# proroklab/magat_pathplanning

Measured on AMD Instinct MI355X. Metric: agent-steps/s (batched GAT forward), higher is better.
Workload: dtype f32 in/out, fp32-class arithmetic: convolutions + GAT maps as f16x3 split products on the 16-bit matrix cores with f32 accumulation (the encoder head too, on the layer3 kernel's pooled map; with GAT_MFMA the attention scores and the K-hop aggregation as well), MLPs on f32 MFMA

## Files before the change

### magat_pathplanning_amd/_native.py

```python
import ctypes
import os
import threading

PKG = os.path.dirname(os.path.abspath(__file__))
LIB_PATH = os.environ.get("MAGAT_LIB_PATH") or os.path.join(PKG, "lib", "libmagat_hip.so")

MODE_KEYQUERY = 0
MODE_GAT_MODIFIED = 1
MODE_GAT_ORIGIN = 2
MODE_GNN = 3
_MODE_IDS = {"KeyQuery": MODE_KEYQUERY, "GAT_modified": MODE_GAT_MODIFIED, "GAT_origin": MODE_GAT_ORIGIN}
TAGS = {0: "untagged", 1: "conv_first", 2: "layer1.conv1", 3: "layer1.conv2+ds", 4: "layer2.conv1",
        5: "layer2.conv2+ds", 6: "layer3.conv1", 7: "layer3.conv2+ds", 8: "head(avgpool+fc+linear)",
        9: "compressMLP", 10: "gat_maps_gemm", 11: "gat_graph", 12: "actionsMLP", 13: "head_mean",
        14: "gat_pack", 15: "gso_prepare", 16: "gat_prepare", 17: "range_guard", 18: "layer1.conv2+layer2 (fused)", 19: "gat_layer (one launch)", 20: "gso_to_csr", 21: "gat_cast", 22: "layer3 (fused, pooled)", 23: "layer1.conv2+layer2+layer3 (fused, pooled)", 24: "conv_wgrad", 25: "gnn_dense", 26: "sim_guided", 27: "sim_expert", 28: "sim_mapf", 29: "sim_mapf_lns", 30: "sim_mapf_audit", 31: "sim_mapf_cbs", 32: "sim_mapf_ecbs"}
TAG_ACTIONS = 12
FORMS = {"head_longk": 0, "head_splitk": 1, "gat_pack": 2, "gat_persist": 3, "gat_hsplit": 4, "chain_persist": 5,
         "head_compress": 6, "guard_one": 7, "csr_fused": 8, "gat_mid": 9, "chain_lat": 10, "head_lat": 11, "guard_lat": 12, "stem_lat": 13, "actions_tail": 14, "gnn_dense": 15, "sim_guided": 16, "sim_expert": 17, "sim_mapf": 18, "sim_mapf_lns": 19, "sim_mapf_audit": 20, "sim_mapf_cbs": 21, "sim_mapf_ecbs": 22}
TAG_GNN_DENSE = 25
TAG_SIM_GUIDED = 26
TAG_SIM_EXPERT = 27
TAG_SIM_MAPF = 28
TAG_SIM_MAPF_LNS = 29
TAG_SIM_MAPF_AUDIT = 30
TAG_SIM_MAPF_CBS = 31
TAG_SIM_MAPF_ECBS = 32
GUIDE_LOCAL, GUIDE_GLOBAL, GUIDE_SEMI = 1, 2, 3

_lock = threading.Lock()
_lib = None


class MagatNativeError(RuntimeError):
# ... 215 lines not shown
```

### magat_pathplanning_amd/csrc/block_fused.hip

```cpp
#include "magat_common.h"

namespace {
#ifndef MAGAT_CHAIN_NT
#define MAGAT_CHAIN_NT 3
#endif
#if MAGAT_CHAIN_NT & 1
#define MAGAT_CHAIN_NT_STR " nt"
#else
#define MAGAT_CHAIN_NT_STR ""
#endif
#if MAGAT_CHAIN_NT & 2
#define CHAIN_OUT_STORE(ptr, val) __builtin_nontemporal_store((val), reinterpret_cast<f32x4*>(ptr))
#else
#define CHAIN_OUT_STORE(ptr, val) (*reinterpret_cast<f32x4*>(ptr) = (val))
#endif
#include "block_walk.h"
struct ChainParams {
  const char* in1;
  const char* in2;
  char* out;
  int out_gl;
  long long out_pix_stride, out_tile;
  const char* wA; const char* wB; const char* wC;
  const float* bA; const float* bB; const float* bC;
// ... 349 lines not shown
    __syncthreads();
    CHAIN_STAMP(3);
    if (more) dma_map(p.in1, group + (int)gridDim.x, LDS_X1N);
    if (rg == 0) chain_stage4<W4A, 32, 0, 64, false>(p, lds, LDS_Y, 0, LDS_Z, p.wB, ct, p.bB, sB, group, clamped);
    else chain_stage4<W4B, 32, 0, 64, false>(p, lds, LDS_Y, 0, LDS_Z, p.wB, ct, p.bB, sB, group, clamped);
    CHAIN_STAMP(4);
    __syncthreads();
    CHAIN_STAMP(5);
    if (rg == 0) chain_stage4<W4A, 64, 32, 64, true>(p, lds, LDS_Z, LDS_Y, 0, p.wC, ct, p.bC, sC, group, clamped);
    else chain_stage4<W4B, 64, 32, 64, true>(p, lds, LDS_Z, LDS_Y, 0, p.wC, ct, p.bC, sC, group, clamped);
    CHAIN_STAMP(6);
  }
  if (clamped && p.range_flag) atomicOr(p.range_flag, 1);
}

struct FullParams { ChainParams c; L3Params l; };



__global__ __launch_bounds__(256, 1) void block_full_p_kernel(const FullParams q) {
  extern __shared__ __attribute__((aligned(1024))) char lds[];
  const ChainParams& p = q.c;
  const L3Params& l3 = q.l;
  const int t = threadIdx.x, lane = t & 63;
  const int wave = __builtin_amdgcn_readfirstlane(t >> 6);
  for (int i = t; i < 32 * (PIXB / 4); i += 256)
    *reinterpret_cast<unsigned*>(lds + (i / (PIXB / 4)) * BLK + ZPIX * PIXB + (i % (PIXB / 4)) * 4) = 0u;
  auto dma_map = [&](const char* base, int group, int lds_off, int first, int step, int last) {
    const int m0 = group * AG;
    const long long tile_b = (long long)(m0 >> 7) * NPIX * (128 * 32 * 4) + (m0 & 127) * 16;
    for (int item = first; item < last; item += step) {
      const int blk = item / 5, part = item % 5;
      const int pix = part * 8 + (lane >> 3);
      const char* src = base + tile_b + (long long)pix * (128 * 32 * 4) + (blk >> 2) * (256 * 32) + (blk & 3) * 2048 +
                        (lane & 7) * 16;
      const unsigned m0v = __builtin_amdgcn_readfirstlane((unsigned)(uintptr_t)lds + (unsigned)(lds_off + blk * BLK + part * 8 * PIXB));
      if (pix < NPIX) asm volatile("s_mov_b32 m0, %1\n\tglobal_load_lds_dwordx4 %0, off" MAGAT_CHAIN_NT_STR ::"v"(src), "s"(m0v) : "memory", "m0");
    }
  };
  const float sA = *p.sA, sB = *p.sB, sC = *p.sC, s1 = *l3.s1, s2 = *l3.s2;
  bool clamped = false;
  const int ct = wave & 1, rg = wave >> 1, ct2 = wave;
  constexpr int BPT1 = 9 * 4 * 2, BPT2A = 9 * 4 * 2, BPT2B = (9 * 4 + 4) * 2;
  f32x4 bq[4];
  {
    const int fh = lane >> 5;
#pragma unroll
    for (int qd = 0; qd < 4; ++qd) bq[qd] = *reinterpret_cast<const f32x4*>(l3.b2 + 32 * ct2 + 8 * qd + 4 * fh);
  }
  FULL_CLOCKS(0);
  const int gstride = (int)gridDim.x;
  constexpr int U0 = 0, U1 = MAP32, U2 = 2 * MAP32, U3 = 3 * MAP32;
  if ((int)blockIdx.x < p.groups) {
    dma_map(p.in1, blockIdx.x, U3, wave, 4, 40);
    dma_map(p.in2, blockIdx.x, U2, wave, 4, 40);
  }
#pragma unroll 1
  for (int group = blockIdx.x; group < p.groups; group += gstride) {
    const bool rows_ok = group * AG + ((lane & 31) & 7) < p.M;
    const bool more = group + gstride < p.groups;
// ... 7 lines not shown
      case 2: chain_stage4<W4P2, 32, 32, 32, false>(p, lds, U3, U2, U1, p.wA, 0, p.bA, sA, group, clamped); break;
      default: chain_stage4<W4P3, 32, 32, 32, false>(p, lds, U3, U2, U1, p.wA, 0, p.bA, sA, group, clamped); break;
    }
    __syncthreads();
    FULL_STAMP(2);
    if (rg == 0) chain_stage4<W4I, 32, 0, 64, false>(p, lds, U1, 0, U2, p.wB, ct, p.bB, sB, group, clamped);
    else chain_stage4<W4E, 32, 0, 64, false>(p, lds, U1, 0, U2, p.wB, ct, p.bB, sB, group, clamped);
    __syncthreads();
    FULL_STAMP(3);
    if (rg == 0) chain_stage4<W4I, 64, 32, 64, false, true>(p, lds, U2, U1, U0, p.wC, ct, p.bC, sC, group, clamped);
    else chain_stage4<W4E, 64, 32, 64, false, true>(p, lds, U2, U1, U0, p.wC, ct, p.bC, sC, group, clamped);
    __syncthreads();
    FULL_STAMP(4);
    constexpr int L_IN = U0, L_MID = U2;
    const int ct1 = ct, rg1 = rg;
    f32x16 acc[9];
#pragma unroll
    for (int s = 0; s < 9; ++s)
#pragma unroll
      for (int r = 0; r < 16; ++r) acc[s][r] = 0.f;
    auto l3_half = [&](const int h) __attribute__((always_inline)) {
      const char* w2 = h == 0 ? l3.w2a + (size_t)ct2 * BPT2A * 1024 : l3.w2b + (size_t)ct2 * BPT2B * 1024;
      const char* w1h = l3.w1 + (size_t)(2 * h) * BPT1 * 1024;
      if (rg1 == 0) {
        f32x16 a1[W4I::NT];
#pragma unroll
        for (int s = 0; s < W4I::NT; ++s)
#pragma unroll
          for (int r = 0; r < 16; ++r) a1[s][r] = 0.f;
        walk4<W4I, 4, 0, 8 * BLK, 8 * BLK, MAGAT_W4_D>(lds, L_IN, 0, w1h + (size_t)ct1 * BPT1 * 1024, a1, false);
        if (h == 0) FULL_STAMP(11); else FULL_STAMP(13);
        const int tl[W4I::NT] = {W4I::t[0], W4I::t[1], W4I::t[2], W4I::t[3]};
        epi_to_lds<64, W4I::NT>(lds, L_MID, tl, a1, ct1, l3.b1 + 64 * h, s1, rows_ok, clamped);
      } else {
        f32x16 a1[W4E::NT];
#pragma unroll
        for (int s = 0; s < W4E::NT; ++s)
#pragma unroll
          for (int r = 0; r < 16; ++r) a1[s][r] = 0.f;
        walk4<W4E, 4, 0, 8 * BLK, 8 * BLK, MAGAT_W4_D>(lds, L_IN, 0, w1h + (size_t)ct1 * BPT1 * 1024, a1, false);
        if (h == 0) FULL_STAMP(11); else FULL_STAMP(13);
        const int tl[W4E::NT] = {W4E::t[0], W4E::t[1], W4E::t[2], W4E::t[3], W4E::t[4]};
        epi_to_lds<64, W4E::NT>(lds, L_MID, tl, a1, ct1, l3.b1 + 64 * h, s1, rows_ok, clamped);
      }
      if (h == 0) FULL_STAMP(12); else FULL_STAMP(14);
      __syncthreads();
      FULL_STAMP(5 + 2 * h);
      walk4<W4All, 4, 4, 8 * BLK, 8 * BLK, MAGAT_W4_D>(lds, L_MID, L_IN, w2, acc, h == 1);
      L3_LDS_SYNC();
      FULL_STAMP(6 + 2 * h);
    };
#if defined(MAGAT_L3_UNROLL_H) && defined(MAGAT_DEBUG_HOOKS)
    l3_half(0);
    l3_half(1);
#else
#pragma unroll 1
    for (int h = 0; h < 2; ++h) l3_half(h);
#endif
    if (more) {
      dma_map(p.in1, group + gstride, U3, wave, 4, 40);
      dma_map(p.in2, group + gstride, U2, wave, 4, 40);
    }
    FULL_STAMP(9);
    {
      const int fr = lane & 31, fh = lane >> 5, agent = fr & 7;
      const bool lo = (lane >> 3) & 1, hi = (lane >> 4) & 1;
      const int m = group * AG + agent;
      const int cellF = 2 * (int)lo + 6 * (int)hi, cell0 = hi ? 1 : 7, cell1 = lo ? 3 : 5;
      float* ob = l3.out + (long long)(m >> 7) * 9 * (128 * 128) +
                  (l3.out_gl ? (8 * ct2 + fh) * 512 + (m & 127) * 4 : (m & 127) * 128 + 32 * ct2 + 4 * fh);
      const int qstep = l3.out_gl ? 1024 : 8;
      const bool mok = m < p.M;
#pragma unroll
      for (int qd = 0; qd < 4; ++qd) {
        f32x4 vF, v0, v1, v2;
#pragma unroll
        for (int c = 0; c < 4; ++c) {
          const int r = 4 * qd + c;
          float v[9];
// ... 99 lines not shown
  }
  const int grid = p.groups < cus ? p.groups : cus;
  hipLaunchKernelGGL(block3_w4_kernel, dim3((unsigned)grid), dim3(256), lds, st, p);
  magat_prof_end(pid, st);
  return magat_check_launch();
}

#ifdef MAGAT_DEBUG_HOOKS
extern "C" int magat_chain_set_debug_buffer(long long* dev_buf) { g_chain_dbg = dev_buf; return MAGAT_OK; }
extern "C" int magat_block3_set_debug_buffer(long long* dev_buf) { g_block3_dbg = dev_buf; return MAGAT_OK; }
#endif


int magat_block_full(const void* in1, const void* in2, const float* wchain, const float* bA, const float* bB, const float* bC,
                     float* out, const float* w3, const float* b1, const float* b2, int M, int* range_flag, hipStream_t st,
                     const float* scales, int out_gl) {
  if (!in1 || !in2 || !wchain || !bA || !bB || !bC || !out || !w3 || !b1 || !b2) return MAGAT_ERR_NULL;
  if (M <= 0) return MAGAT_ERR_BAD_SHAPE;
  FullParams q;
  ChainParams& p = q.c;
  p.in1 = static_cast<const char*>(in1); p.in2 = static_cast<const char*>(in2); p.out = nullptr;
  p.out_gl = 2; p.out_pix_stride = 0; p.out_tile = 0;
  const char* wb = reinterpret_cast<const char*>(wchain);
  const size_t nA = chain_block_bytes(32, 32, 32), nB = chain_block_bytes(32, 0, 64), nC = chain_block_bytes(64, 32, 64);
  p.wA = wb; p.wB = wb + nA + 16; p.wC = wb + nA + 16 + nB + 16;
  p.bA = bA; p.bB = bB; p.bC = bC;
  p.sA = reinterpret_cast<const float*>(p.wA + nA);
  p.sB = reinterpret_cast<const float*>(p.wB + nB);
  p.sC = reinterpret_cast<const float*>(p.wC + nC);
  p.M = M; p.groups = (M + AG - 1) / AG;
  p.range_flag = range_flag;
// ... 3 lines not shown
  const char* w3b = reinterpret_cast<const char*>(w3);
  const size_t n1 = (size_t)4 * 72 * 1024, n2a = (size_t)4 * 72 * 1024, n2b = (size_t)4 * 80 * 1024;
  l.w1 = w3b; l.w2a = w3b + n1 + 16; l.w2b = w3b + n1 + 16 + n2a + 16;
  l.s1 = reinterpret_cast<const float*>(l.w1 + n1);
  l.s2 = reinterpret_cast<const float*>(l.w2b + n2b);
  l.b1 = b1; l.b2 = b2;
  if (scales) { p.sA = scales; p.sB = scales + 1; p.sC = scales + 2; l.s1 = scales + 3; l.s2 = scales + 4; }
  l.M = M; l.groups = p.groups;
  l.range_flag = range_flag;
  l.dbg = nullptr;
#ifdef MAGAT_DEBUG_HOOKS
  l.dbg = g_block3_dbg;
#endif
  if (out_gl != 0 && out_gl != 1) return MAGAT_ERR_UNSUPPORTED;
  l.out_gl = out_gl;
  if (magat_ensure_dyn_lds(reinterpret_cast<const void*>(&block_full_p_kernel), MAGAT_LDS_BLOCK_FULL_P, LDS_TOTAL) != MAGAT_OK)
    return MAGAT_ERR_LAUNCH;
  int dev = 0, cus = 256;
  if (hipGetDevice(&dev) == hipSuccess) {
    int v = 0;
    if (hipDeviceGetAttribute(&v, hipDeviceAttributeMultiprocessorCount, dev) == hipSuccess && v > 0) cus = v;
  }
  const int grid = p.groups < cus ? p.groups : cus;
  if (p.groups > cus) magat_form_note(MAGAT_FORM_CHAIN_PERSIST);
  const int pid = magat_prof_begin(MAGAT_TAG_BLOCK_FULL, st);
  hipLaunchKernelGGL(block_full_p_kernel, dim3((unsigned)grid), dim3(256), LDS_TOTAL, st, q);
  magat_prof_end(pid, st);
  return magat_check_launch();
}
```

### magat_pathplanning_amd/csrc/block_walk.h

```cpp
#pragma once
#include "f16x3.h"

constexpr int AG = 8;
constexpr int NPIX = 36, ZPIX = 36;
constexpr int PIXB = AG * 16;
constexpr int BLK = (NPIX + 1) * PIXB;
constexpr int MAP32 = 8 * BLK;
constexpr int MAP64 = 16 * BLK;
constexpr int LDS_X2 = MAP32, LDS_Z = 0, LDS_Y = MAP64, LDS_X1N = MAP64 + MAP32, LDS_TOTAL = MAP64 + 2 * MAP32;
constexpr int TAPBIAS = 7 * PIXB;

__device__ constexpr int TILE_PIX[9][4] = {{7, 10, 25, 28},  {26, 27, 8, 9},   {16, 13, 22, 19}, {14, 15, 20, 21},
                                           {1, 4, 2, 3},     {32, 33, 31, 34}, {6, 12, 24, 18},  {17, 11, 23, 29},
                                           {0, 5, 30, 35}};
__device__ __forceinline__ int tile_pix(int tile, int psl) {
  const unsigned packed = (unsigned)TILE_PIX[tile][0] | (unsigned)TILE_PIX[tile][1] << 8 | (unsigned)TILE_PIX[tile][2] << 16 |
                          (unsigned)TILE_PIX[tile][3] << 24;
  return (int)((packed >> (8 * psl)) & 0xFFu);
}
__device__ constexpr int TILE_TAPS[9] = {0x1FF, 0x1FF, 0x1FF, 0x1FF, 0x1F8, 0x03F, 0x1B6, 0x0DB, 0x1FF};
constexpr int T_I0 = 0, T_I1 = 1, T_I2 = 2, T_I3 = 3, T_ET = 4, T_EB = 5, T_EL = 6, T_ER = 7, T_C = 8;
__device__ constexpr int WT32[8][3] = {{T_I0, -1, -1}, {T_I2, -1, -1}, {T_C, -1, -1},  {T_EB, T_EL, -1},
                                       {T_I1, -1, -1}, {T_I3, -1, -1}, {T_ET, -1, -1}, {T_ER, -1, -1}};
__device__ constexpr int WG64[4][3] = {{T_I0, T_I1, -1}, {T_I2, T_I3, -1}, {T_C, T_ET, -1}, {T_EB, T_EL, T_ER}};
// ... 148 lines not shown
    acc[it.s] = __builtin_amdgcn_mfma_f32_32x32x16_f16(__builtin_bit_cast(f16x8, w[step % D][1]),
                                                       __builtin_bit_cast(f16x8, av[i % AV][0]), acc[it.s], 0, 0, 0);
    W4_PIN();
    if (more) { if (more_ok) rd(SQ.it[more ? i + LA : i], 1, av[(i + LA) % AV][1]); W4_PIN(); }
    acc[it.s] = __builtin_amdgcn_mfma_f32_32x32x16_f16(__builtin_bit_cast(f16x8, w[step % D][0]),
                                                       __builtin_bit_cast(f16x8, av[i % AV][1]), acc[it.s], 0, 0, 0);
    W4_PIN();
  }
}


struct W4P0 { static constexpr int NT = 2; static constexpr int t[2] = {T_I0, T_I1}; };
struct W4P1 { static constexpr int NT = 2; static constexpr int t[2] = {T_I2, T_I3}; };
struct W4P2 { static constexpr int NT = 2; static constexpr int t[2] = {T_C, T_ET}; };
struct W4P3 { static constexpr int NT = 3; static constexpr int t[3] = {T_EB, T_EL, T_ER}; };
```

### magat_pathplanning_amd/csrc/encoder_f32.hip

```cpp
#include <cstdlib>

#include "magat_common.h"

namespace {

template <int HC, int WC>
__global__ __launch_bounds__(256) void conv_first_kernel(const float* __restrict__ x, const float* __restrict__ wt,
                                                         const float* __restrict__ bias, float* __restrict__ out,
                                                         int M, int Hr, int Wr, long long out_pix_stride,
                                                         long long out_tile_stride, long long out_plane, int out_gl,
                                                         int* range_flag, const int* run_if, int BH, float* absmax) {
  extern __shared__ float img[];
  if (run_if && *run_if == 0) return;
  const int H = HC ? HC : Hr, W = WC ? WC : Wr;
  const int BHe = HC ? HC : BH;
  const int ybase = HC ? 0 : (int)blockIdx.y * BHe;
  const int bh = min(BHe, H - ybase);
  const int PW = W + 2, PHW = (BHe + 2) * PW;
  const int PS = (3 * PHW) | 1;
  const int HW = H * W;
  const int t = threadIdx.x, lane = t & 63, wave = t >> 6;
  float amax = 0.f;
  for (int blk = blockIdx.x; blk * 32 < M; blk += gridDim.x) {
  if (blk != (int)blockIdx.x) __syncthreads();
// ... 388 lines not shown
        lg.x = x + (size_t)m0 * 3 * H * W; lg.pack = pk; lg.off = d->off; lg.book = reinterpret_cast<int*>(range_flag);
      }
      if (lat_all && !(lat && head_done)) return MAGAT_ERR_UNSUPPORTED;
      if (lat) {
        rc = magat_block_lat(buf[1], buf[0], pk + d->chain_off, sp ? sp + 928 : pk + d->off[5], sp ? sp + 960 : pk + d->off[7],
                             sp ? sp + 1024 : pk + d->off[9], buf[2], pk + d->chain3_off, sp ? sp + 1088 : pk + d->off[11],
                             sp ? sp + 1216 : pk + d->off[13], mm, reinterpret_cast<int*>(range_flag), st,
                             sp ? sp + 1344 : nullptr, head_gl ? 1 : 0, head_done ? &lh : nullptr, inguard ? &lg : nullptr,
                             (lat_all && head_done) ? &ls : nullptr);
        if (rc != MAGAT_OK) return rc;
        if (inguard) *self_guarded = true;
      } else
        rc = magat_block_full(buf[1], buf[0], pk + d->chain_off, sp ? sp + 928 : pk + d->off[5], sp ? sp + 960 : pk + d->off[7],
                              sp ? sp + 1024 : pk + d->off[9], buf[2], pk + d->chain3_off, sp ? sp + 1088 : pk + d->off[11],
                              sp ? sp + 1216 : pk + d->off[13], mm, reinterpret_cast<int*>(range_flag), st, sp ? sp + 1344 : nullptr,
                              head_gl ? 1 : 0);
      if (rc != MAGAT_OK) return rc;
      cur = 2; hin = Ho; win = Wo; lstart = 3; pooled_in = true;
    } else if (fused1 && d->chain_off > 0 && Ho == 6 && Wo == 6 && nblocks >= 2 && magat_opt(MAGAT_OPT_BLOCK_FUSED)) {
      rc = magat_block_chain(buf[1], buf[0], buf[2], nblocks == 2 ? 0 : 2, pixs(64), tiles(Ho * Wo, 64), pk + d->chain_off,
                             pk + d->off[5], pk + d->off[7], pk + d->off[9], mm, reinterpret_cast<int*>(range_flag), st);
      if (rc != MAGAT_OK) return rc;
      cur = 2; hin = Ho; win = Wo; lstart = 2;
      if (nblocks == 3 && d->chain3_off > 0) {
        rc = magat_block3(buf[2], buf[0], pk + d->chain3_off, pk + d->off[11], pk + d->off[13], mm,
                          reinterpret_cast<int*>(range_flag), st);
        if (rc != MAGAT_OK) return rc;
        cur = 0; lstart = 3; pooled_in = true;
      }
    }
    for (int l = lstart; l < nblocks; ++l) {
// ... 260 lines not shown
```

### magat_pathplanning_amd/csrc/magat_common.h

```cpp
#pragma once
#include <hip/hip_runtime.h>
#include <stdint.h>

#include "../../include/magat_hip.h"

typedef float f32x2 __attribute__((ext_vector_type(2)));
typedef float f32x4 __attribute__((ext_vector_type(4)));
typedef float f32x16 __attribute__((ext_vector_type(16)));

#if (defined(MAGAT_WHATIF_NO_W) || defined(MAGAT_WHATIF_NO_LDS) || defined(CSR_WHATIF_NODMA) || defined(CSR_WHATIF_NOLOOP) || defined(CSR_WHATIF_NOIDX) || defined(CSR_WHATIF_NOKLOOP) || defined(CSR_WHATIF_NOSTORE) || \
     defined(GM_WHATIF_NOQW) || defined(GM_WHATIF_NOAW) || defined(GM_WHATIF_NOYST) || defined(FUSED_WHATIF_COALESCED) || defined(FUSED_WHATIF_NOSCALAR)) && !defined(MAGAT_EXPERIMENT_BUILD)
#error "*_WHATIF_* timing switches produce wrong results: they compile only with -DMAGAT_EXPERIMENT_BUILD (see magat_common.h)"
#endif
extern "C" int magat_experiment_mark(void);
#ifdef MAGAT_EXPERIMENT_BUILD
namespace { struct MagatExperimentMark { MagatExperimentMark() { magat_experiment_mark(); } } g_magat_experiment_mark; }
#endif

#define MAGAT_WAVE 64
#define MAGAT_TILE_ROWS 128
__host__ __device__ __forceinline__ long long magat_row_off(long long m, long long ld, long long tile_stride) {
  return (m >> 7) * tile_stride + (m & 127) * ld;
}
#define MAGAT_NUM_XCD 8
// ... 6 lines not shown
#define MAGAT_TAG_SIM_MAPF 28
#define MAGAT_PROF_TAGS_ALL 29
#define MAGAT_FORM_SIM_GUIDED 16
#define MAGAT_FORM_SIM_EXPERT 17
#define MAGAT_FORM_SIM_MAPF 18
#define MAGAT_FORMS_ALL 19
#define MAGAT_TAG_SIM_MAPF_LNS 29
#define MAGAT_TAG_SIM_MAPF_AUDIT 30
#define MAGAT_TAG_SIM_MAPF_CBS 31
#define MAGAT_TAG_SIM_MAPF_ECBS 32
#define MAGAT_PROF_TAGS_TABLE 33
#define MAGAT_FORM_SIM_MAPF_LNS 19
#define MAGAT_FORM_SIM_MAPF_AUDIT 20
#define MAGAT_FORM_SIM_MAPF_CBS 21
#define MAGAT_FORM_SIM_MAPF_ECBS 22
#define MAGAT_FORMS_TABLE 23
static_assert(MAGAT_PROF_TAGS_ALL >= MAGAT_PROF_TAGS && MAGAT_FORMS_ALL >= MAGAT_FORMS, "internal tag / form tables");
static_assert(MAGAT_PROF_TAGS_TABLE > MAGAT_TAG_SIM_MAPF_ECBS && MAGAT_PROF_TAGS_TABLE >= MAGAT_PROF_TAGS_ALL &&
              MAGAT_FORMS_TABLE > MAGAT_FORM_SIM_MAPF_ECBS && MAGAT_FORMS_TABLE >= MAGAT_FORMS_ALL, "internal tag / form tables");

int magat_conv_gemm_bf16x6(const magat_conv_gemm_desc* d, hipStream_t st);
int magat_layer1_fused(const float* x, const float* w0, const float* b0, const float* w1, const float* b1, void* out,
                       void* ctr, int M, int H, int W, hipStream_t st, int* range_flag = nullptr);
size_t magat_layer1_fused_lds(int W);
int magat_stem8(const float* x, const float* w0, const float* b0, const float* w1f, const float* b1, void* out, void* ctr,
                int M, int H, int W, hipStream_t st, int* range_flag = nullptr);
size_t magat_block_chain_weight_floats();
size_t magat_block3_weight_floats();
int magat_block_full(const void* in1, const void* in2, const float* wchain, const float* bA, const float* bB, const float* bC,
                     float* out, const float* w3, const float* b1, const float* b2, int M, int* range_flag, hipStream_t st,
                     const float* scales = nullptr,
                     int out_gl = 0);
int magat_block_full_out_gl();
struct magat_lat_head {
  const float* hfrag; const float* cfrag;
  const float* hbias; const float* cbias;
  const float* insc; const float* insc2;
  float* feat; int ldfeat; float* comp; int ldcomp;
  int ncomp;
};
struct magat_lat_guard {
  const float* x;
  const float* pack; const int64_t* off;
  int* book;
};
struct magat_lat_stem {
  const float* x;
// ... 5 lines not shown
                    const float* scales = nullptr, int out_gl = 0, const magat_lat_head* head = nullptr,
                    const magat_lat_guard* guard = nullptr, const magat_lat_stem* stem = nullptr);
int magat_block3(const void* in, float* out, const float* w, const float* b1, const float* b2, int M, int* range_flag,
                 hipStream_t st);
int magat_block_chain(const void* in1, const void* in2, void* out, int out_gl, long long out_pix_stride, long long out_tile,
                      const float* w, const float* bA, const float* bB, const float* bC, int M, int* range_flag,
                      hipStream_t st);
int magat_conv_direct_enabled();
int magat_conv_gemm_chain_f32(const magat_conv_gemm_desc* descs, int n, const int32_t* run_if, int tag, hipStream_t st,
                              int32_t* book = nullptr);

enum MagatOpt {
  MAGAT_OPT_ENC_CHUNK, MAGAT_OPT_CONV_SPLIT, MAGAT_OPT_CONV_PCHAIN,
  MAGAT_OPT_L1_FUSED, MAGAT_OPT_HEAD_SPLITK, MAGAT_OPT_GAT_CHUNK_MB, MAGAT_OPT_GAT_SPLIT, MAGAT_OPT_RANGE_GUARD,
  MAGAT_OPT_BLOCK_FUSED, MAGAT_OPT_CSR_TILED, MAGAT_OPT_HEAD_F16, MAGAT_OPT_GAT_MFMA, MAGAT_OPT_SKINNY, MAGAT_OPT_GAT_PACK,
  MAGAT_OPT_CONV_BNFILL, MAGAT_OPT_HEAD_COMPRESS, MAGAT_OPT_CONV_TM, MAGAT_OPT_CSR_FUSED, MAGAT_OPT_LAT_AGENTS, MAGAT_OPT_GAT_WIDE_FROM, MAGAT_OPT_COUNT
};
int magat_opt(int id);
#define MAGAT_LDS_SLOTS 192
int magat_ensure_dyn_lds(const void* func, int slot, size_t bytes);
enum MagatLdsSlot {
  MAGAT_LDS_GAT16, MAGAT_LDS_GAT32, MAGAT_LDS_GAT64, MAGAT_LDS_GAT128, MAGAT_LDS_GAT256, MAGAT_LDS_L1FUSED,
  MAGAT_LDS_SIM_GSO_T, MAGAT_LDS_SIM_GSO_F, MAGAT_LDS_SIM_MOVE, MAGAT_LDS_BLOCK_A, MAGAT_LDS_BLOCK_B, MAGAT_LDS_BLOCK_C,
  MAGAT_LDS_SIM_CONN, MAGAT_LDS_CONV_FIRST, MAGAT_LDS_CONV_FIRST11, MAGAT_LDS_GSO_STRUCT, MAGAT_LDS_CSR_TILED_A, MAGAT_LDS_CSR_TILED_B, MAGAT_LDS_CSR_TILED_A16, MAGAT_LDS_CSR_TILED_B16,
  MAGAT_LDS_CSR_TILED_A4, MAGAT_LDS_CSR_TILED_B4, MAGAT_LDS_CSR_TILED_A16_4, MAGAT_LDS_CSR_TILED_B16_4, MAGAT_LDS_BLOCK_B4, MAGAT_LDS_BLOCK_FULL, MAGAT_LDS_BLOCK_FULL_P, MAGAT_LDS_BLOCK_FULL_C, MAGAT_LDS_BLOCK_FULL_C4, MAGAT_LDS_BLOCK_FULL_C5,
  MAGAT_LDS_GATM_0,
  MAGAT_LDS_GATM_END = MAGAT_LDS_GATM_0 + 24,
  MAGAT_LDS_STEM8,
  MAGAT_LDS_GATP_0,
  MAGAT_LDS_GATP_END = MAGAT_LDS_GATP_0 + 8,
  MAGAT_LDS_GATS_0,
  MAGAT_LDS_GATS_END = MAGAT_LDS_GATS_0 + 8,
  MAGAT_LDS_CSR_FUSED_A,
  MAGAT_LDS_CSR_FUSED_B = MAGAT_LDS_CSR_FUSED_A + 3,
  MAGAT_LDS_CSR_FUSED_END = MAGAT_LDS_CSR_FUSED_B + 2,
  MAGAT_LDS_GATD_0 = MAGAT_LDS_CSR_FUSED_END,
  MAGAT_LDS_GATD_END = MAGAT_LDS_GATD_0 + 56,
  MAGAT_LDS_BLOCK_LAT, MAGAT_LDS_BLOCK_LAT_H, MAGAT_LDS_BLOCK_LAT_S,
  MAGAT_LDS_GAT_SLIM,
  MAGAT_LDS_GAT_RERUN_S, MAGAT_LDS_GAT_RERUN_S_END = MAGAT_LDS_GAT_RERUN_S + 5,
  MAGAT_LDS_GNND_0,
  MAGAT_LDS_GNND_END = MAGAT_LDS_GNND_0 + 5,
  MAGAT_LDS_SIM_MAPF = MAGAT_LDS_GNND_END,
  MAGAT_LDS_SIM_MOVE_WIDE,
  MAGAT_LDS_SIM_MAPF_LNS,
  MAGAT_LDS_SIM_MAPF_CBS,
  MAGAT_LDS_END
};
static_assert(MAGAT_LDS_END <= MAGAT_LDS_SLOTS, "LDS attribute slots");

int magat_gat_csr_fused_supported(int G, int F, int K, int P, int mode, int concat);
int magat_gat_csr_fused_pack(const float* Bt, void* frag_out, int P, hipStream_t st);
size_t magat_gat_csr_fused_order_bytes(int B, int N);
int magat_gat_csr_fused_forward(const uint16_t* X, const int* rowptr, const int* colidx, const int* cscptr, const int* cscsrc,
                                const int* cscpos, long long nnz, const void* frags, const float* bias, void* Y, int ldy,
                                int y_f32, float* att , float* att_opt , int* order, int B, int N,
                                int P, hipStream_t st);
int magat_cast_rows_if(const void* src, void* dst, int to_bf16, long long M, int width, int ld_src, int ld_dst, void* stream,
                       const int32_t* run_if);
int magat_gat_small_supported(int N, int G, int F, int K, int mode);
int magat_gat_small_forward(const float* X, int ldx, const void* S, int s_is_f64, const unsigned* rmask_pre, const float* Hs,
// ... 98 lines not shown
```

### magat_pathplanning_amd/csrc/options.hip

```cpp
#include <atomic>
#include <cstdlib>
#include <cstring>
#include <mutex>

#include "magat_common.h"

namespace {

struct OptEntry {
  const char* name;
  int def;
};

const OptEntry kOpts[MAGAT_OPT_COUNT] = {
    {"ENC_CHUNK", 65536},
    {"CONV_SPLIT", 7},
    {"CONV_PCHAIN", 1},
    {"L1_FUSED", 2},
    {"HEAD_SPLITK", 5120},
    {"GAT_CHUNK_MB", 2048},
    {"GAT_SPLIT", 1},
    {"RANGE_GUARD", 1},
    {"BLOCK_FUSED", 2},
    {"CSR_TILED", 3},
    {"HEAD_F16", 1},
    {"GAT_MFMA", 1},
    {"SKINNY", 1},
    {"GAT_PACK", 1},
    {"CONV_BNFILL", 256},
    {"HEAD_COMPRESS", 1},
    {"CONV_TM", 2},
    {"CSR_FUSED", 1},
    {"LAT_AGENTS", 512},
    {"GAT_WIDE_FROM", 103},
};

int g_val[MAGAT_OPT_COUNT];
int g_start[MAGAT_OPT_COUNT];
std::once_flag g_once;

void init_opts() {
  for (int i = 0; i < MAGAT_OPT_COUNT; ++i) {
    g_val[i] = kOpts[i].def;
    char key[64] = "MAGAT_";
    strncat(key, kOpts[i].name, sizeof(key) - 7);
    const char* e = getenv(key);
    if (e && *e) g_val[i] = atoi(e);
    g_start[i] = g_val[i];
  }
// ... 68 lines not shown
```

### magat_pathplanning_amd/encoder.py

```python
import math

import torch

BN_EPS = 1e-5


def _bn_scale_shift(sd, pre):
    s = sd[pre + ".weight"].double() / torch.sqrt(sd[pre + ".running_var"].double() + BN_EPS)
    return s, sd[pre + ".bias"].double() - sd[pre + ".running_mean"].double() * s


def _conv_rows(w, scale):
    co = w.shape[0]
    return (w.double() * scale.view(-1, 1, 1, 1)).permute(0, 2, 3, 1).reshape(co, -1)


def fold_resnet(sd, H=11, W=11, pre="ConvLayers.0", linear=None, compress=None):
    sd = {k: v.detach().cpu() for k, v in sd.items() if k.startswith(pre)}
    parts, offs = [], [0] * 32
    cursor = [0]

    def put(slot, t):
        t = t.reshape(-1)
        offs[slot] = cursor[0]
# ... 88 lines not shown
    if Ho == 6 and Wo == 6 and nblocks >= 2:
        def rows(slot, cout):
            nxt = sorted(o for o in offs[:18] if o > offs[slot])
            return pack[offs[slot]:(nxt[0] if nxt else n_f32)].reshape(cout, -1)
        blocks = [pack_chain_weights(rows(4, 32)[:, :9 * 32 + 32], 32, 32),
                  pack_chain_weights(rows(6, 64)[:, :9 * 32], 32, 0),
                  pack_chain_weights(rows(8, 64)[:, :9 * 64 + 32], 64, 32)]
        chain_off = pack.numel()
        pack = torch.cat([pack] + blocks).contiguous()
    chain3_off = 0
    if chain_off and large:
        def rows3(slot):
            nxt = sorted(o for o in offs[:18] if o > offs[slot])
            return pack[offs[slot]:(nxt[0] if nxt else n_f32)].reshape(128, -1)
        chain3_off = pack.numel()
        pack = torch.cat([pack] + pack_block3_weights(rows3(10)[:, :9 * 64], rows3(12)[:, :9 * 128 + 64])).contiguous()
    nxt = sorted(o for o in offs[:18] if o > offs[14])
    head16, _ = split_f16x2(pack[offs[14]:(nxt[0] if nxt else n_f32)])
    pad = (-head16.numel()) % 4
    if pad:
        head16 = torch.cat((head16, torch.zeros(pad)))
    head16_off = pack.numel()
    pack = torch.cat([pack, head16]).contiguous()
    comp16_off = 0
    if n_comp > 0:
        comp16, _ = split_f16x2(pack[offs[16]:offs[16] + n_comp * n_feat])
        pad = (-comp16.numel()) % 4
        if pad:
            comp16 = torch.cat((comp16, torch.zeros(pad)))
        comp16_off = pack.numel()
        pack = torch.cat([pack, comp16]).contiguous()
# ... 1 lines not shown
    if chain3_off and n_comp in (32, 64, 128) and n_feat == 128 and clast == 128 and Hp * Wp == 9:
        nxt = sorted(o for o in offs[:18] if o > offs[14])
        hrows = pack[offs[14]:(nxt[0] if nxt else n_f32)].reshape(n_feat, Hp * Wp * clast)
        hsteps = [cell * clast + 32 * cs + 16 * ks for cs in range(clast // 32) for cell in range(Hp * Wp) for ks in range(2)]
        headfrag_off = pack.numel()
        pack = torch.cat([pack, pack_frag_natural(hrows, hsteps)]).contiguous()
        crows = pack[offs[16]:offs[16] + n_comp * n_feat].reshape(n_comp, n_feat)
        compfrag_off = pack.numel()
        pack = torch.cat([pack, pack_frag_natural(crows, [16 * ks for ks in range(n_feat // 16)])]).contiguous()
    l1frag_off = 0
    if H == 11 and W == 11:
        nxt = sorted(o for o in offs[:18] if o > offs[2])
        w1rows = pack[offs[2]:(nxt[0] if nxt else n_f32)][:32 * 288].reshape(32, 288)
        l1frag_off = pack.numel()
        pack = torch.cat([pack, pack_chain_weights(w1rows, 32, 0)]).contiguous()
    meta = dict(variant=0 if large else 1, H=H, W=W, n_feat=n_feat, n_comp=n_comp, clast=clast, chain=chain_off,
                chain3=chain3_off, head16=head16_off, comp16=comp16_off, l1frag=l1frag_off, headfrag=headfrag_off,
                compfrag=compfrag_off)
    return pack, offs, meta


SCALED_BLOCK_FLOATS = 1352


def scale_exponent(m, target_log2=10, lo=-14, hi=24):
    if not (m > 0.0) or not math.isfinite(m):
        return 0
    return max(lo, min(hi, target_log2 - int(math.floor(math.log2(m))) - 1))


# ... 32 lines not shown
    blk[1348] = s32 * f(-s3)
    blk[1349] = f(e_head)
    blk[1350] = f(e_feat)
    return blk.to(torch.float32), dict(s1=s1, s2=s2, s3=s3, head_in=e_head, feat_in=e_feat)


def pack_block3_weights(w1, w2):
    w2 = w2.detach().float().cpu()
    taps = w2[:, :9 * 128].reshape(128, 9, 128)
    lo = taps[:, :, :64].reshape(128, 9 * 64)
    hi = torch.cat((taps[:, :, 64:].reshape(128, 9 * 64), w2[:, 9 * 128:]), dim=1)
    mx = float(w2.abs().max())
    e = 0 if mx == 0.0 else 13 - int(math.floor(math.log2(mx)))
    e = max(-14, min(e, 24))
    return [pack_chain_weights(w1, 64, 0), pack_chain_weights(lo, 64, 0, e=e), pack_chain_weights(hi, 64, 64, e=e)]


def chain_channel(ks, fh, i):
    return 32 * (ks >> 1) + 16 * (ks & 1) + 8 * (i >> 2) + 4 * fh + (i & 3)


def pack_chain_weights(w, cin, c2, e=None):
    w = w.detach().float().cpu()
    cout = w.shape[0]
    assert w.shape[1] == 9 * cin + c2 and cout % 32 == 0 and cin % 16 == 0 and c2 % 16 == 0
    if e is None:
        mx = float(w.abs().max())
        e = 0 if mx == 0.0 else 13 - int(math.floor(math.log2(mx)))
        e = max(-14, min(e, 24))
    ws = w * (2.0 ** e)
# ... 170 lines not shown
```

Before: 22.31 million.

## Add 16x16 half-tile MFMA path for fused layer3 conv in block_full kernel

```diff
diff --git a/magat_pathplanning_amd/_native.py b/magat_pathplanning_amd/_native.py
--- a/magat_pathplanning_amd/_native.py
+++ b/magat_pathplanning_amd/_native.py
@@ -16,7 +16,8 @@
         14: "gat_pack", 15: "gso_prepare", 16: "gat_prepare", 17: "range_guard", 18: "layer1.conv2+layer2 (fused)", 19: "gat_layer (one launch)", 20: "gso_to_csr", 21: "gat_cast", 22: "layer3 (fused, pooled)", 23: "layer1.conv2+layer2+layer3 (fused, pooled)", 24: "conv_wgrad", 25: "gnn_dense", 26: "sim_guided", 27: "sim_expert", 28: "sim_mapf", 29: "sim_mapf_lns", 30: "sim_mapf_audit", 31: "sim_mapf_cbs", 32: "sim_mapf_ecbs"}
 TAG_ACTIONS = 12
 FORMS = {"head_longk": 0, "head_splitk": 1, "gat_pack": 2, "gat_persist": 3, "gat_hsplit": 4, "chain_persist": 5,
-         "head_compress": 6, "guard_one": 7, "csr_fused": 8, "gat_mid": 9, "chain_lat": 10, "head_lat": 11, "guard_lat": 12, "stem_lat": 13, "actions_tail": 14, "gnn_dense": 15, "sim_guided": 16, "sim_expert": 17, "sim_mapf": 18, "sim_mapf_lns": 19, "sim_mapf_audit": 20, "sim_mapf_cbs": 21, "sim_mapf_ecbs": 22}
+         "head_compress": 6, "guard_one": 7, "csr_fused": 8, "gat_mid": 9, "chain_lat": 10, "head_lat": 11, "guard_lat": 12, "stem_lat": 13, "actions_tail": 14, "gnn_dense": 15, "sim_guided": 16, "sim_expert": 17, "sim_mapf": 18, "sim_mapf_lns": 19, "sim_mapf_audit": 20, "sim_mapf_cbs": 21, "sim_mapf_ecbs": 22,
+         "chain_tile16": 23}
 TAG_GNN_DENSE = 25
 TAG_SIM_GUIDED = 26
 TAG_SIM_EXPERT = 27
diff --git a/magat_pathplanning_amd/csrc/block_fused.hip b/magat_pathplanning_amd/csrc/block_fused.hip
--- a/magat_pathplanning_amd/csrc/block_fused.hip
+++ b/magat_pathplanning_amd/csrc/block_fused.hip
@@ -387,10 +387,14 @@
   if (clamped && p.range_flag) atomicOr(p.range_flag, 1);
 }
 
-struct FullParams { ChainParams c; L3Params l; };
-
-
-
+struct FullParams {
+  ChainParams c; L3Params l;
+  const char* w2a16; const char* w2b16;
+};
+
+
+
+template <bool T16>
 __global__ __launch_bounds__(256, 1) void block_full_p_kernel(const FullParams q) {
   extern __shared__ __attribute__((aligned(1024))) char lds[];
   const ChainParams& p = q.c;
@@ -416,7 +420,10 @@
   const int ct = wave & 1, rg = wave >> 1, ct2 = wave;
   constexpr int BPT1 = 9 * 4 * 2, BPT2A = 9 * 4 * 2, BPT2B = (9 * 4 + 4) * 2;
   f32x4 bq[4];
-  {
+  if constexpr (T16) {
+#pragma unroll
+    for (int hf = 0; hf < 2; ++hf) bq[hf] = *reinterpret_cast<const f32x4*>(l3.b2 + 32 * ct2 + 16 * hf + 4 * (lane >> 4));
+  } else {
     const int fh = lane >> 5;
 #pragma unroll
     for (int qd = 0; qd < 4; ++qd) bq[qd] = *reinterpret_cast<const f32x4*>(l3.b2 + 32 * ct2 + 8 * qd + 4 * fh);
@@ -454,13 +461,22 @@
     FULL_STAMP(4);
     constexpr int L_IN = U0, L_MID = U2;
     const int ct1 = ct, rg1 = rg;
-    f32x16 acc[9];
-#pragma unroll
-    for (int s = 0; s < 9; ++s)
-#pragma unroll
-      for (int r = 0; r < 16; ++r) acc[s][r] = 0.f;
+    f32x16 acc[T16 ? 1 : 9];
+    f32x4 acc16[2][T16 ? HT_N : 1];
+    if constexpr (T16) {
+#pragma unroll
+      for (int hf = 0; hf < 2; ++hf)
+#pragma unroll
+        for (int s = 0; s < HT_N; ++s) acc16[hf][s] = f32x4{0.f, 0.f, 0.f, 0.f};
+    } else {
+#pragma unroll
+      for (int s = 0; s < 9; ++s)
+#pragma unroll
+        for (int r = 0; r < 16; ++r) acc[s][r] = 0.f;
+    }
     auto l3_half = [&](const int h) __attribute__((always_inline)) {
-      const char* w2 = h == 0 ? l3.w2a + (size_t)ct2 * BPT2A * 1024 : l3.w2b + (size_t)ct2 * BPT2B * 1024;
+      const char* w2 = h == 0 ? (T16 ? q.w2a16 : l3.w2a) + (size_t)ct2 * BPT2A * 1024
+                              : (T16 ? q.w2b16 : l3.w2b) + (size_t)ct2 * BPT2B * 1024;
       const char* w1h = l3.w1 + (size_t)(2 * h) * BPT1 * 1024;
       if (rg1 == 0) {
         f32x16 a1[W4I::NT];
@@ -486,7 +502,8 @@
       if (h == 0) FULL_STAMP(12); else FULL_STAMP(14);
       __syncthreads();
       FULL_STAMP(5 + 2 * h);
-      walk4<W4All, 4, 4, 8 * BLK, 8 * BLK, MAGAT_W4_D>(lds, L_MID, L_IN, w2, acc, h == 1);
+      if constexpr (T16) walk16<2, 2, 8 * BLK, 8 * BLK, 3>(lds, L_MID, L_IN, w2, acc16, h == 1);
+      else walk4<W4All, 4, 4, 8 * BLK, 8 * BLK, MAGAT_W4_D>(lds, L_MID, L_IN, w2, acc, h == 1);
       L3_LDS_SYNC();
       FULL_STAMP(6 + 2 * h);
     };
@@ -502,7 +519,44 @@
       dma_map(p.in2, group + gstride, U2, wave, 4, 40);
     }
     FULL_STAMP(9);
-    {
+    if constexpr (T16) {
+      const int agent = lane & 7, kq = lane >> 4;
+      const bool sl = (lane >> 3) & 1;
+      const int m = group * AG + agent;
+      const int cellA = sl ? 2 : 0, cellB = sl ? 8 : 6, cellE = sl ? 3 : 5;
+      const bool mok = m < p.M;
+#pragma unroll
+      for (int hf = 0; hf < 2; ++hf) {
+        const int g = 8 * ct2 + 4 * hf + kq;
+        float* ob = l3.out + (long long)(m >> 7) * 9 * (128 * 128) + (l3.out_gl ? g * 512 + (m & 127) * 4 : (m & 127) * 128 + 4 * g);
+        f32x4 vA, vB, vE, v1, v7, v4;
+#pragma unroll
+        for (int c = 0; c < 4; ++c) {
+          float v[HT_N];
+#pragma unroll
+          for (int s = 0; s < HT_N; ++s) v[s] = magat_relu(__builtin_fmaf(acc16[hf][s][c], s2, bq[hf][c]));
+          const float ea = sl ? v[HT_RA] : v[HT_LA], eb = sl ? v[HT_RB] : v[HT_LB];
+          const float xa = sl ? v[HT_LA] : v[HT_RA], xb = sl ? v[HT_LB] : v[HT_RB];
+          vA[c] = (v[HT_CT] + v[HT_I1]) + (v[HT_TA] + ea);
+          vB[c] = (v[HT_CB] + v[HT_I2]) + (v[HT_BA] + eb);
+          vE[c] = (v[HT_I5] + v[HT_I6]) + (xa + xb);
+          const float p1 = v[HT_TB] + v[HT_I3], p7 = v[HT_BB] + v[HT_I4], p4 = v[HT_I7] + v[HT_I8];
+          v1[c] = p1 + dpp_mov<0x128>(p1);
+          v7[c] = p7 + dpp_mov<0x128>(p7);
+          v4[c] = p4 + dpp_mov<0x128>(p4);
+        }
+        if (mok) {
+          CHAIN_OUT_STORE(ob + (long long)cellA * (128 * 128), vA);
+          CHAIN_OUT_STORE(ob + (long long)cellB * (128 * 128), vB);
+          CHAIN_OUT_STORE(ob + (long long)cellE * (128 * 128), vE);
+          if (!sl) {
+            CHAIN_OUT_STORE(ob + (long long)1 * (128 * 128), v1);
+            CHAIN_OUT_STORE(ob + (long long)7 * (128 * 128), v7);
+            CHAIN_OUT_STORE(ob + (long long)4 * (128 * 128), v4);
+          }
+        }
+      }
+    } else {
       const int fr = lane & 31, fh = lane >> 5, agent = fr & 7;
       const bool lo = (lane >> 3) & 1, hi = (lane >> 4) & 1;
       const int m = group * AG + agent;
@@ -632,7 +686,7 @@
 
 int magat_block_full(const void* in1, const void* in2, const float* wchain, const float* bA, const float* bB, const float* bC,
                      float* out, const float* w3, const float* b1, const float* b2, int M, int* range_flag, hipStream_t st,
-                     const float* scales, int out_gl) {
+                     const float* scales, int out_gl, const float* w3t16, int Mform) {
   if (!in1 || !in2 || !wchain || !bA || !bB || !bC || !out || !w3 || !b1 || !b2) return MAGAT_ERR_NULL;
   if (M <= 0) return MAGAT_ERR_BAD_SHAPE;
   FullParams q;
@@ -666,7 +720,13 @@
 #endif
   if (out_gl != 0 && out_gl != 1) return MAGAT_ERR_UNSUPPORTED;
   l.out_gl = out_gl;
-  if (magat_ensure_dyn_lds(reinterpret_cast<const void*>(&block_full_p_kernel), MAGAT_LDS_BLOCK_FULL_P, LDS_TOTAL) != MAGAT_OK)
+  const int t16opt = magat_opt(MAGAT_OPT_CHAIN_TILE16);
+  const bool t16 = t16opt == 1 || (t16opt >= 2 && w3t16 && (Mform > 0 ? Mform : M) >= MAGAT_CHAIN_TILE16_FROM);
+  if (t16 && !w3t16) return MAGAT_ERR_UNSUPPORTED;
+  q.w2a16 = t16 ? reinterpret_cast<const char*>(w3t16) : nullptr;
+  q.w2b16 = t16 ? reinterpret_cast<const char*>(w3t16) + n2a : nullptr;
+  const void* kfn = t16 ? reinterpret_cast<const void*>(&block_full_p_kernel<true>) : reinterpret_cast<const void*>(&block_full_p_kernel<false>);
+  if (magat_ensure_dyn_lds(kfn, t16 ? MAGAT_LDS_BLOCK_FULL_P16 : MAGAT_LDS_BLOCK_FULL_P, LDS_TOTAL) != MAGAT_OK)
     return MAGAT_ERR_LAUNCH;
   int dev = 0, cus = 256;
   if (hipGetDevice(&dev) == hipSuccess) {
@@ -676,7 +736,11 @@
   const int grid = p.groups < cus ? p.groups : cus;
   if (p.groups > cus) magat_form_note(MAGAT_FORM_CHAIN_PERSIST);
   const int pid = magat_prof_begin(MAGAT_TAG_BLOCK_FULL, st);
-  hipLaunchKernelGGL(block_full_p_kernel, dim3((unsigned)grid), dim3(256), LDS_TOTAL, st, q);
+  if (t16) {
+    magat_form_note(MAGAT_FORM_CHAIN_TILE16);
+    hipLaunchKernelGGL(block_full_p_kernel<true>, dim3((unsigned)grid), dim3(256), LDS_TOTAL, st, q);
+  } else
+    hipLaunchKernelGGL(block_full_p_kernel<false>, dim3((unsigned)grid), dim3(256), LDS_TOTAL, st, q);
   magat_prof_end(pid, st);
   return magat_check_launch();
 }
diff --git a/magat_pathplanning_amd/csrc/block_walk.h b/magat_pathplanning_amd/csrc/block_walk.h
--- a/magat_pathplanning_amd/csrc/block_walk.h
+++ b/magat_pathplanning_amd/csrc/block_walk.h
@@ -186,3 +186,146 @@
 struct W4P1 { static constexpr int NT = 2; static constexpr int t[2] = {T_I2, T_I3}; };
 struct W4P2 { static constexpr int NT = 2; static constexpr int t[2] = {T_C, T_ET}; };
 struct W4P3 { static constexpr int NT = 3; static constexpr int t[3] = {T_EB, T_EL, T_ER}; };
+
+
+constexpr int HT_N = 18;
+constexpr int HT_PIX[HT_N][2] = {{7, 10},  {25, 28}, {8, 9},   {26, 27}, {16, 13}, {22, 19}, {14, 15}, {20, 21},
+                                 {0, 5},   {30, 35},
+                                 {1, 4},   {2, 3},   {31, 34}, {32, 33},
+                                 {6, 12},  {24, 18}, {17, 11}, {23, 29}};
+constexpr int HT_TAPS[HT_N] = {0x1FF, 0x1FF, 0x1FF, 0x1FF, 0x1FF, 0x1FF, 0x1FF, 0x1FF, 0x1F8, 0x03F,
+                               0x1F8, 0x1F8, 0x03F, 0x03F, 0x1B6, 0x1B6, 0x0DB, 0x0DB};
+constexpr int HT_I1 = 0, HT_I2 = 1, HT_I3 = 2, HT_I4 = 3, HT_I5 = 4, HT_I6 = 5, HT_I7 = 6, HT_I8 = 7, HT_CT = 8, HT_CB = 9,
+              HT_TA = 10, HT_TB = 11, HT_BA = 12, HT_BB = 13, HT_LA = 14, HT_LB = 15, HT_RA = 16, HT_RB = 17;
+constexpr bool ht_tap_valid(int pix, int tp) {
+  const int y = pix / 6 + tp / 3 - 1, x = pix % 6 + tp % 3 - 1;
+  return y >= 0 && y < 6 && x >= 0 && x < 6;
+}
+constexpr bool ht_tables_ok() {
+  int seen[NPIX] = {}, taps = 0;
+  for (int s = 0; s < HT_N; ++s) {
+    for (int sl = 0; sl < 2; ++sl) seen[HT_PIX[s][sl]] += 1;
+    for (int tp = 0; tp < 9; ++tp) {
+      const bool v0 = ht_tap_valid(HT_PIX[s][0], tp), v1 = ht_tap_valid(HT_PIX[s][1], tp);
+      const bool run = HT_TAPS[s] >> tp & 1;
+      if (run != (v0 || v1)) return false;
+      if (run && v0 != v1 && s != HT_CT && s != HT_CB) return false;
+      taps += run;
+    }
+  }
+  for (int pix = 0; pix < NPIX; ++pix)
+    if (seen[pix] != 1) return false;
+  return taps == 132;
+}
+static_assert(ht_tables_ok(), "half tiles: pixels, tap masks or the tap count");
+constexpr int h16_minshift(int s) {
+  int m = 99;
+  for (int tp = 0; tp < 9; ++tp)
+    if (HT_TAPS[s] >> tp & 1) {
+      const int sh = 6 * (tp / 3 - 1) + (tp % 3 - 1);
+      if (sh < m) m = sh;
+    }
+  return m;
+}
+template <int KSM, int KS2>
+constexpr W4Seq<(132 * KSM + HT_N * KS2) + 1> h16_seq() {
+  W4Seq<(132 * KSM + HT_N * KS2) + 1> q{};
+  int n = 0;
+  for (int tp = 0; tp < 9; ++tp)
+    for (int ks = 0; ks < KSM; ++ks) {
+      bool first = true;
+      for (int s = 0; s < HT_N; ++s)
+        if (HT_TAPS[s] >> tp & 1) {
+          q.it[n].tp = (signed char)tp; q.it[n].ks = (signed char)ks; q.it[n].s = (signed char)s; q.it[n].first = first;
+          first = false;
+          ++n;
+        }
+    }
+  q.nmain = n;
+  for (int ks = 0; ks < KS2; ++ks)
+    for (int s = 0; s < HT_N; ++s) {
+      q.it[n].tp = 9; q.it[n].ks = (signed char)ks; q.it[n].s = (signed char)s; q.it[n].first = s == 0;
+      ++n;
+    }
+  q.n = n;
+  return q;
+}
+template <int KSM, int KS2, int PS_IN, int PS_IN2, int D>
+__device__ __forceinline__ void walk16(char* lds, int in_off, int in2_off, const char* wbase, f32x4 (&acc)[2][HT_N], bool with_res) {
+  u32x4 w[D][4];
+  constexpr auto SQ = h16_seq<KSM, KS2>();
+  constexpr int NMAIN = 9 * KSM, NSTEP = NMAIN + KS2;
+  int tid = threadIdx.x;
+  asm volatile("" : "+v"(tid));
+  const int lane = tid & 63;
+  const unsigned lane16 = (unsigned)lane * 16u;
+  const int agent = lane & 7, sl = (lane >> 3) & 1, kq = lane >> 4;
+  unsigned ab[HT_N], b0[HT_N];
+  int cmask[2] = {0, 0};
+#pragma unroll
+  for (int s = 0; s < HT_N; ++s) {
+    const int pix = sl ? HT_PIX[s][1] : HT_PIX[s][0];
+    ab[s] = (unsigned)(pix * PIXB + agent * 16 + kq * BLK);
+    b0[s] = ab[s] + (unsigned)(in_off + h16_minshift(s) * PIXB);
+    asm volatile("" : "+v"(b0[s]));
+    if (s == HT_CT || s == HT_CB) {
+      const int y = pix / 6, x = pix - 6 * y;
+#pragma unroll
+      for (int tp = 0; tp < 9; ++tp) {
+        const int dy = tp / 3 - 1, dx = tp % 3 - 1;
+        if (y + dy >= 0 && y + dy < 6 && x + dx >= 0 && x + dx < 6) cmask[s - HT_CT] |= 1 << tp;
+      }
+    }
+  }
+  const unsigned az = (unsigned)(ZPIX * PIXB + agent * 16 + kq * BLK + in_off);
+  auto load_w = [&](int step, u32x4 (&b)[4]) {
+#pragma unroll
+    for (int j = 0; j < 4; ++j) b[j] = *reinterpret_cast<const u32x4*>(wbase + (size_t)step * 4096 + (lane16 + 1024u * j));
+  };
+  constexpr int AV = MAGAT_W4_AV;
+  u32x4 av[AV][2];
+  auto rd = [&](const W4Item it, int pl, u32x4& dst) {
+    if (it.tp == 9) {
+      dst = *reinterpret_cast<const u32x4*>(lds + (ab[it.s] + (unsigned)in2_off) + (pl * PS_IN2 + it.ks * 4 * BLK));
+    } else if (it.s == HT_CT || it.s == HT_CB) {
+      const int sh = 6 * (it.tp / 3 - 1) + (it.tp % 3 - 1);
+      const unsigned a = (cmask[it.s - HT_CT] >> it.tp & 1) ? ab[it.s] + (unsigned)(in_off + sh * PIXB) : az;
+      dst = *reinterpret_cast<const u32x4*>(lds + a + (pl * PS_IN + it.ks * 4 * BLK));
+    } else {
+      const int sh = 6 * (it.tp / 3 - 1) + (it.tp % 3 - 1) - h16_minshift(it.s);
+      dst = *reinterpret_cast<const u32x4*>(lds + b0[it.s] + (sh * PIXB + pl * PS_IN + it.ks * 4 * BLK));
+    }
+  };
+#pragma unroll
+  for (int j = 0; j < D - 1; ++j)
+    if (j < NSTEP) load_w(j, w[j]);
+#pragma unroll
+  for (int j = 0; j < AV - 1; ++j) {
+    rd(SQ.it[j], 0, av[j][0]);
+    rd(SQ.it[j], 1, av[j][1]);
+  }
+#pragma clang loop unroll(full)
+  for (int i = 0; i < SQ.n; ++i) {
+    const W4Item it = SQ.it[i];
+    if (KS2 > 0 && i == SQ.nmain && !with_res) break;
+    const int step = it.tp * KSM + it.ks;
+    if (it.first && step + D - 1 < NSTEP) {
+      if (step + D - 1 < NMAIN || with_res) load_w(step + D - 1, w[(step + D - 1) % D]);
+    }
+    constexpr int LA = AV - 1;
+    const bool more = i + LA < SQ.n;
+    const bool more_ok = more && (i + LA < SQ.nmain || with_res);
+    const f16x8 a0 = __builtin_bit_cast(f16x8, av[i % AV][0]), a1 = __builtin_bit_cast(f16x8, av[i % AV][1]);
+    acc[0][it.s] = __builtin_amdgcn_mfma_f32_16x16x32_f16(__builtin_bit_cast(f16x8, w[step % D][0]), a0, acc[0][it.s], 0, 0, 0);
+    acc[1][it.s] = __builtin_amdgcn_mfma_f32_16x16x32_f16(__builtin_bit_cast(f16x8, w[step % D][2]), a0, acc[1][it.s], 0, 0, 0);
+    W4_PIN();
+    if (more) { if (more_ok) rd(SQ.it[more ? i + LA : i], 0, av[(i + LA) % AV][0]); W4_PIN(); }
+    acc[0][it.s] = __builtin_amdgcn_mfma_f32_16x16x32_f16(__builtin_bit_cast(f16x8, w[step % D][1]), a0, acc[0][it.s], 0, 0, 0);
+    acc[1][it.s] = __builtin_amdgcn_mfma_f32_16x16x32_f16(__builtin_bit_cast(f16x8, w[step % D][3]), a0, acc[1][it.s], 0, 0, 0);
+    W4_PIN();
+    if (more) { if (more_ok) rd(SQ.it[more ? i + LA : i], 1, av[(i + LA) % AV][1]); W4_PIN(); }
+    acc[0][it.s] = __builtin_amdgcn_mfma_f32_16x16x32_f16(__builtin_bit_cast(f16x8, w[step % D][0]), a1, acc[0][it.s], 0, 0, 0);
+    acc[1][it.s] = __builtin_amdgcn_mfma_f32_16x16x32_f16(__builtin_bit_cast(f16x8, w[step % D][2]), a1, acc[1][it.s], 0, 0, 0);
+    W4_PIN();
+  }
+}
diff --git a/magat_pathplanning_amd/csrc/encoder_f32.hip b/magat_pathplanning_amd/csrc/encoder_f32.hip
--- a/magat_pathplanning_amd/csrc/encoder_f32.hip
+++ b/magat_pathplanning_amd/csrc/encoder_f32.hip
@@ -426,7 +426,7 @@
         rc = magat_block_full(buf[1], buf[0], pk + d->chain_off, sp ? sp + 928 : pk + d->off[5], sp ? sp + 960 : pk + d->off[7],
                               sp ? sp + 1024 : pk + d->off[9], buf[2], pk + d->chain3_off, sp ? sp + 1088 : pk + d->off[11],
                               sp ? sp + 1216 : pk + d->off[13], mm, reinterpret_cast<int*>(range_flag), st, sp ? sp + 1344 : nullptr,
-                              head_gl ? 1 : 0);
+                              head_gl ? 1 : 0, d->off[31] > 0 ? pk + d->off[31] : nullptr, Mform);
       if (rc != MAGAT_OK) return rc;
       cur = 2; hin = Ho; win = Wo; lstart = 3; pooled_in = true;
     } else if (fused1 && d->chain_off > 0 && Ho == 6 && Wo == 6 && nblocks >= 2 && magat_opt(MAGAT_OPT_BLOCK_FUSED)) {
diff --git a/magat_pathplanning_amd/csrc/magat_common.h b/magat_pathplanning_amd/csrc/magat_common.h
--- a/magat_pathplanning_amd/csrc/magat_common.h
+++ b/magat_pathplanning_amd/csrc/magat_common.h
@@ -44,10 +44,11 @@
 #define MAGAT_FORM_SIM_MAPF_AUDIT 20
 #define MAGAT_FORM_SIM_MAPF_CBS 21
 #define MAGAT_FORM_SIM_MAPF_ECBS 22
-#define MAGAT_FORMS_TABLE 23
+#define MAGAT_FORM_CHAIN_TILE16 23
+#define MAGAT_FORMS_TABLE 24
 static_assert(MAGAT_PROF_TAGS_ALL >= MAGAT_PROF_TAGS && MAGAT_FORMS_ALL >= MAGAT_FORMS, "internal tag / form tables");
 static_assert(MAGAT_PROF_TAGS_TABLE > MAGAT_TAG_SIM_MAPF_ECBS && MAGAT_PROF_TAGS_TABLE >= MAGAT_PROF_TAGS_ALL &&
-              MAGAT_FORMS_TABLE > MAGAT_FORM_SIM_MAPF_ECBS && MAGAT_FORMS_TABLE >= MAGAT_FORMS_ALL, "internal tag / form tables");
+              MAGAT_FORMS_TABLE > MAGAT_FORM_CHAIN_TILE16 && MAGAT_FORMS_TABLE >= MAGAT_FORMS_ALL, "internal tag / form tables");
 
 int magat_conv_gemm_bf16x6(const magat_conv_gemm_desc* d, hipStream_t st);
 int magat_layer1_fused(const float* x, const float* w0, const float* b0, const float* w1, const float* b1, void* out,
@@ -60,7 +61,10 @@
 int magat_block_full(const void* in1, const void* in2, const float* wchain, const float* bA, const float* bB, const float* bC,
                      float* out, const float* w3, const float* b1, const float* b2, int M, int* range_flag, hipStream_t st,
                      const float* scales = nullptr,
-                     int out_gl = 0);
+                     int out_gl = 0,
+                     const float* w3t16 = nullptr,
+                     int Mform = 0);
+#define MAGAT_CHAIN_TILE16_FROM 10240
 int magat_block_full_out_gl();
 struct magat_lat_head {
   const float* hfrag; const float* cfrag;
@@ -96,7 +100,8 @@
   MAGAT_OPT_ENC_CHUNK, MAGAT_OPT_CONV_SPLIT, MAGAT_OPT_CONV_PCHAIN,
   MAGAT_OPT_L1_FUSED, MAGAT_OPT_HEAD_SPLITK, MAGAT_OPT_GAT_CHUNK_MB, MAGAT_OPT_GAT_SPLIT, MAGAT_OPT_RANGE_GUARD,
   MAGAT_OPT_BLOCK_FUSED, MAGAT_OPT_CSR_TILED, MAGAT_OPT_HEAD_F16, MAGAT_OPT_GAT_MFMA, MAGAT_OPT_SKINNY, MAGAT_OPT_GAT_PACK,
-  MAGAT_OPT_CONV_BNFILL, MAGAT_OPT_HEAD_COMPRESS, MAGAT_OPT_CONV_TM, MAGAT_OPT_CSR_FUSED, MAGAT_OPT_LAT_AGENTS, MAGAT_OPT_GAT_WIDE_FROM, MAGAT_OPT_COUNT
+  MAGAT_OPT_CONV_BNFILL, MAGAT_OPT_HEAD_COMPRESS, MAGAT_OPT_CONV_TM, MAGAT_OPT_CSR_FUSED, MAGAT_OPT_LAT_AGENTS, MAGAT_OPT_GAT_WIDE_FROM,
+  MAGAT_OPT_CHAIN_TILE16, MAGAT_OPT_COUNT
 };
 int magat_opt(int id);
 #define MAGAT_LDS_SLOTS 192
@@ -127,6 +132,7 @@
   MAGAT_LDS_SIM_MOVE_WIDE,
   MAGAT_LDS_SIM_MAPF_LNS,
   MAGAT_LDS_SIM_MAPF_CBS,
+  MAGAT_LDS_BLOCK_FULL_P16,
   MAGAT_LDS_END
 };
 static_assert(MAGAT_LDS_END <= MAGAT_LDS_SLOTS, "LDS attribute slots");
diff --git a/magat_pathplanning_amd/csrc/options.hip b/magat_pathplanning_amd/csrc/options.hip
--- a/magat_pathplanning_amd/csrc/options.hip
+++ b/magat_pathplanning_amd/csrc/options.hip
@@ -33,6 +33,7 @@
     {"CSR_FUSED", 1},
     {"LAT_AGENTS", 512},
     {"GAT_WIDE_FROM", 103},
+    {"CHAIN_TILE16", 2},
 };
 
 int g_val[MAGAT_OPT_COUNT];
diff --git a/magat_pathplanning_amd/encoder.py b/magat_pathplanning_amd/encoder.py
--- a/magat_pathplanning_amd/encoder.py
+++ b/magat_pathplanning_amd/encoder.py
@@ -126,7 +126,8 @@
             nxt = sorted(o for o in offs[:18] if o > offs[slot])
             return pack[offs[slot]:(nxt[0] if nxt else n_f32)].reshape(128, -1)
         chain3_off = pack.numel()
-        pack = torch.cat([pack] + pack_block3_weights(rows3(10)[:, :9 * 64], rows3(12)[:, :9 * 128 + 64])).contiguous()
+        blocks3 = pack_block3_weights(rows3(10)[:, :9 * 64], rows3(12)[:, :9 * 128 + 64])
+        pack = torch.cat([pack] + blocks3).contiguous()
     nxt = sorted(o for o in offs[:18] if o > offs[14])
     head16, _ = split_f16x2(pack[offs[14]:(nxt[0] if nxt else n_f32)])
     pad = (-head16.numel()) % 4
@@ -158,6 +159,9 @@
         w1rows = pack[offs[2]:(nxt[0] if nxt else n_f32)][:32 * 288].reshape(32, 288)
         l1frag_off = pack.numel()
         pack = torch.cat([pack, pack_chain_weights(w1rows, 32, 0)]).contiguous()
+    if chain3_off:
+        offs[31] = pack.numel()
+        pack = torch.cat([pack, pack_block3_tile16(blocks3)]).contiguous()
     meta = dict(variant=0 if large else 1, H=H, W=W, n_feat=n_feat, n_comp=n_comp, clast=clast, chain=chain_off,
                 chain3=chain3_off, head16=head16_off, comp16=comp16_off, l1frag=l1frag_off, headfrag=headfrag_off,
                 compfrag=compfrag_off)
@@ -220,6 +224,16 @@
     e = 0 if mx == 0.0 else 13 - int(math.floor(math.log2(mx)))
     e = max(-14, min(e, 24))
     return [pack_chain_weights(w1, 64, 0), pack_chain_weights(lo, 64, 0, e=e), pack_chain_weights(hi, 64, 64, e=e)]
+
+
+def pack_block3_tile16(blocks):
+    out = []
+    for blk in blocks[1:3]:
+        h = blk[:-4].contiguous().view(torch.int16)
+        s16 = h.numel() // (4 * 2 * 64 * 8)
+        assert s16 % 2 == 0 and h.numel() == 4 * s16 * 1024
+        out.append(h.view(4, s16 // 2, 2, 2, 2, 2, 16, 8).permute(0, 1, 5, 3, 2, 4, 6, 7).contiguous().view(-1).view(torch.float32))
+    return torch.cat(out)
 
 
 def chain_channel(ks, fh, i):
```

Measured after the change: 22.62 million, median of 6. 1.4% higher.
